# DanecLacey/basic_iterative_solvers

Hardware: AMD Instinct MI355X
Metric: CG iterations/sec + SpMV GFLOP/s (% HBM roofline), HPCG 256^3 at 1/2/4/8 GPUs (higher is better)
Workload: dtype f64

## Files before the change

### basic_iterative_solvers_amd/csrc/bis_blas1.hip

```cpp
#include "bis_internal.hpp"

#include <algorithm>
#include <cstdlib>

namespace {

constexpr int kEwThreads = 256;
constexpr int kMaxEwBlocks = 16384;

inline int ew_grid(int64_t n_items) {
    int64_t g = (n_items + kEwThreads - 1) / kEwThreads;
    if (g < 1) g = 1;
    if (g > kMaxDotBlocks) g = kMaxDotBlocks;
    return (int)g;
}
inline int ew_grid_wide(int64_t n_items) {
    int64_t g = (n_items + kEwThreads - 1) / kEwThreads;
    if (g < 1) g = 1;
    if (g > kMaxEwBlocks) g = kMaxEwBlocks;
    return (int)g;
}

typedef double ew_v2d_t __attribute__((ext_vector_type(2)));
__device__ __forceinline__ double2 ld_stream(const double2 *p) {
// ... 130 lines not shown
    int64_t i = (int64_t)blockIdx.x * kEwThreads + threadIdx.x;
    double acc0 = 0.0, acc1 = 0.0;
    if (VEC) {
        const int64_t n2 = n >> 1;
        double2 *w2 = reinterpret_cast<double2 *>(w);
        const double2 *u2 = reinterpret_cast<const double2 *>(u);
        const double2 *v2 = reinterpret_cast<const double2 *>(v);
        for (; i < n2; i += stride) {
            double2 wv = ld_stream(w2 + i);
            const double2 uv = ld_stream(u2 + i);
            wv.x = ew_apply<OP_SUB>(wv.x, uv.x, s);
            wv.y = ew_apply<OP_SUB>(wv.y, uv.y, s);
            w2[i] = wv;
            const double2 vv = v ? ld_stream(v2 + i) : wv;
            acc0 = fma(wv.x, vv.x, acc0);
            acc1 = fma(wv.y, vv.y, acc1);
        }
        if ((n & 1) && blockIdx.x == 0 && threadIdx.x == 0) {
            const double t = ew_apply<OP_SUB>(w[n - 1], u[n - 1], s);
            w[n - 1] = t;
            acc0 = fma(t, v ? v[n - 1] : t, acc0);
        }
    } else {
        for (; i < n; i += stride) {
            const double t = ew_apply<OP_SUB>(w[i], u[i], s);
            w[i] = t;
            acc0 = fma(t, v ? v[i] : t, acc0);
        }
    }
    const double r = block_sum<kEwThreads>(acc0 + acc1, lds);
    if (threadIdx.x == 0) partials[blockIdx.x] = r;
}

__global__ __launch_bounds__(256) void reduce_finish_kernel(const double *partials,
                                                            int n_partials, size_t stride,
                                                            double *result) {
    __shared__ double lds[4];
    const double *p = partials + (size_t)blockIdx.x * stride;
    double acc = 0.0;
    for (int i = threadIdx.x; i < n_partials; i += 256) acc += p[i];
    const double s = block_sum<256>(acc, lds);
    if (threadIdx.x == 0) result[blockIdx.x] = s;
}

enum { SC_DIV, SC_RATIO_PRODUCT, SC_SQRT_INV };
__global__ void scalar_kernel(int op, double *out, double *out2, const double *a, const double *b, const double *c,
                              const double *d) {
    if (op == SC_DIV) *out = *a / *b;
    else if (op == SC_RATIO_PRODUCT) *out = (*a / *b) * (*c / *d);
    else { const double nrm = sqrt(*a); *out = nrm; *out2 = 1.0 / nrm; }
}

}

bis_status bis_reduce_finish(bis_ctx *ctx, int n_partials, int n_values, size_t stride,
                             double *result_dev) {
    hipLaunchKernelGGL(reduce_finish_kernel, dim3(n_values), dim3(256), 0, ctx->stream,
                       ctx->partials, n_partials, stride, result_dev);
    BIS_HIP_CHECK(ctx, hipGetLastError());
    return BIS_OK;
}

bis_status bis_ensure_partials(bis_ctx *ctx, size_t n) {
    if (n <= ctx->partials_cap) return BIS_OK;
    BIS_HIP_CHECK(ctx, hipStreamSynchronize(ctx->stream));
    if (ctx->partials) BIS_HIP_CHECK(ctx, hipFree(ctx->partials));
    ctx->partials = nullptr;
    ctx->partials_cap = 0;
    BIS_HIP_CHECK(ctx, hipMalloc(&ctx->partials, sizeof(double) * n));
    ctx->partials_cap = n;
    return BIS_OK;
}

bis_status bis_fault_check(bis_ctx *ctx) {
    volatile unsigned *f = ctx->fault_host;
    if (!f || *f == 0) return BIS_OK;
    *f = 0;
    ctx->err = "a triangular sweep lost a hand-off: a row waited for a result that was never published "
               "(a workgroup of the persistent grid could not become resident, or the dependency data is corrupt); "
               "the vectors written since the last blocking call are invalid";
    return BIS_ERR_SYNC;
}

#define BIS_OPTIONS_ENV(X) X(spmv_variant) X(spmv_window) X(spmv_chunk) X(spmv_chunk_fused) X(spmv_xcd_remap) X(trsv_grid) X(ilu0_wgs) X(trsv_wave_wgs) X(trsv_trial) X(trsv_one_xcd) X(trsv_host_analysis) X(ilu0_wave) X(spmv_packed) X(spmv_packed32) X(spmv_valdict) X(spmv_sellwin) X(device_share) X(spmv_sellwin_rows) X(spmv_sellwin_joint) X(spmv_sellwin_pairs) X(spmv_sellwin_masks) X(spmv_colslab) X(spmv_win8) X(spmv_win8_rows) X(spmv_win8_depth) X(spmv_win8_implicit) X(spmv_win8_tune) X(spmv_win4) X(grid_autodetect) X(tune_placement) X(force_rp64) X(trsv_tiled) X(trsv_chain) X(trsv_tile_rows) X(trsv_tile_wgs) X(trsv_tile_edge) X(trsv_tile_backoff)
#define BIS_OPTIONS_API(Y) Y(trsv_batch) Y(trsv_wave) Y(ilu0_persistent) Y(trsv_by_pos) Y(spmv_lds_pad) Y(trsv_chain_idle) Y(trsv_chain_pause) Y(trsv_chain_pairs) Y(trsv_chain_prefix) Y(trsv_tile_exp) Y(cg_nt_x) Y(spmv_sellwin_nt) Y(dist_host_plan) Y(trsv_inject_loss) Y(trsv_inject_oom) Y(trsm_form)

namespace {
std::string &opts_env_seen() { static std::string s; return s; }
std::string upper_env(const char *name) {
    std::string e = "BIS_";
    for (const char *c = name; *c; ++c) e += (char)((*c >= 'a' && *c <= 'z') ? *c - 32 : *c);
    return e;
}
}

bis_options &bis_opts() {
    static bis_options o = [] {
        bis_options v;
#define X(name) { const std::string en = upper_env(#name); if (const char *e = getenv(en.c_str())) { v.name = atoi(e); \
                  std::string &seen = opts_env_seen(); if (!seen.empty()) seen += ' '; seen += en + "=" + e; } }
        BIS_OPTIONS_ENV(X)
#undef X
        return v;
    }();
    return o;
}

extern "C" {

bis_status bis_set_option(const char *name, int value) {
    if (!name) return BIS_ERR_INVALID;
    bis_options &o = bis_opts();
#define X(opt) if (!strcmp(name, #opt)) { o.opt = value; return BIS_OK; }
    BIS_OPTIONS_ENV(X)
    BIS_OPTIONS_API(X)
#undef X
    return BIS_ERR_INVALID;
}

int bis_options_describe(char *buf, int cap) {
    const bis_options &o = bis_opts();
    std::string s = "{";
    bool first = true;
#define X(opt) if (o.opt != -1) { if (!first) s += ", "; first = false; s += std::string("\"") + #opt + "\": " + std::to_string(o.opt); }
    BIS_OPTIONS_ENV(X)
    BIS_OPTIONS_API(X)
#undef X
    if (!first) s += ", ";
    s += "\"env\": \"";
    for (char c : opts_env_seen()) if (c != '"' && c != '\\' && (unsigned char)c >= 32) s += c;
    s += "\"}";
    if (buf && cap > 0) { const int n = std::min((int)s.size(), cap - 1); memcpy(buf, s.data(), (size_t)n); buf[n] = 0; }
    return (int)s.size();
}

int bis_abi_version(void) { return 1; }

bis_status bis_ctx_create(int device, void *stream, bis_ctx **out) {
    if (!out) return BIS_ERR_INVALID;
    *out = nullptr;
    int count = 0;
    if (hipGetDeviceCount(&count) != hipSuccess || count <= 0) return BIS_ERR_NO_DEVICE;
    if (device < 0 || device >= count) return BIS_ERR_NO_DEVICE;
    if (hipSetDevice(device) != hipSuccess) return BIS_ERR_NO_DEVICE;
    hipDeviceProp_t prop;
    if (hipGetDeviceProperties(&prop, device) != hipSuccess) return BIS_ERR_NO_DEVICE;
    bis_ctx *ctx = new bis_ctx;
    ctx->device = device;
    ctx->n_cus = prop.multiProcessorCount;
    ctx->arch = prop.gcnArchName;
    ctx->hbm_bytes = (int64_t)prop.totalGlobalMem;
    if (ctx->arch.rfind("gfx950", 0) != 0) {
        fprintf(stderr, "bis_hip: device %d is %s, this library is built for gfx950 only\n",
                device, ctx->arch.c_str());
        delete ctx;
        return BIS_ERR_NO_DEVICE;
    }
    if (stream) {
        ctx->stream = (hipStream_t)stream;
    } else {
        if (hipStreamCreateWithFlags(&ctx->stream, hipStreamNonBlocking) != hipSuccess) {
            delete ctx;
            return BIS_ERR_HIP;
        }
        ctx->own_stream = true;
    }
    ctx->partials_cap = std::max((size_t)kMaxReduceBlocks * 4, (size_t)kMaxDotBlocks * 2);
// ... 327 lines not shown
```

### basic_iterative_solvers_amd/csrc/bis_internal.hpp

```cpp
#pragma once

#include <hip/hip_runtime.h>

#include <cstdint>
#include <cstdio>
#include <cstring>
#include <map>
#include <string>
#include <vector>

#include "bis_hip.h"

struct bis_trsv_plan;
struct bis_trsv_tiled;
struct bis_trsv_chain;
struct bis_trsm_plan;
struct bis_trsv_side {
    bis_trsv_plan *level = nullptr;
    bis_trsv_tiled *tiled = nullptr;
    bis_trsv_chain *chain = nullptr;
    bis_trsm_plan *multi = nullptr;
    bool tiled_tried = false, chain_tried = false;
    const char *kernel = "";
    const char *kernel_m = "";
// ... 3 lines not shown
    int type = 0;
    const bis_mat *A = nullptr;
    double *B = nullptr, *C = nullptr;
    int64_t size_B = 0, size_C = 0;
    const double *D = nullptr;
    bool upper = false;
};

struct bis_ctx {
    int device = 0;
    hipStream_t stream = nullptr;
    bool own_stream = false;
    int n_cus = 0;
    std::string arch;
    int64_t hbm_bytes = 0;
    std::string err;

    double *partials = nullptr;
    size_t partials_cap = 0;
    double *scalars_dev = nullptr;
    double *scalars_host = nullptr;
    unsigned *counters = nullptr;
    unsigned *fault_host = nullptr, *fault_dev = nullptr;

    std::map<std::string, bis_named_kernel> kernels;

    const int *spmv_stop = nullptr;

    bool profile = false;
    std::vector<std::pair<hipEvent_t, hipEvent_t>> prof_events;
    size_t prof_used = 0;
    std::vector<std::pair<hipEvent_t, hipEvent_t>> prof_sweep_events;
    size_t prof_sweep_used = 0;
};

struct bis_options;
bis_options &bis_opts();
struct bis_options {
    int spmv_variant = -1;
    int spmv_window = -1;
    int spmv_chunk = -1;
    int spmv_chunk_fused = -1;
    int spmv_xcd_remap = -1;
    int trsv_grid = -1;
    int ilu0_wave = -1;
    int ilu0_wgs = -1;
    int ilu0_persistent = -1;
    int trsv_host_analysis = -1;
    int trsv_wave = -1;
    int trsv_wave_wgs = -1;
    int trsv_trial = -1;
    int trsv_batch = -1;
    int trsv_by_pos = -1;
    int trsv_one_xcd = -1;
    int tune_placement = -1;
    int spmv_packed32 = -1;
    int spmv_lds_pad = -1;
    int spmv_packed = -1;
    int spmv_valdict = -1;
    int dist_host_plan = -1;
    int grid_autodetect = -1;
    int trsv_chain = -1;
    int trsv_chain_idle = -1;
    int trsv_chain_pause = -1;
    int trsv_chain_prefix = -1;
    int trsv_chain_pairs = -1;
    int trsv_tiled = -1;
    int trsv_tile_rows = -1;
    int trsv_tile_wgs = -1;
    int trsv_tile_backoff = -1;
    int spmv_sellwin_nt = -1;
    int cg_nt_x = -1;
    int trsv_tile_exp = -1;
    int trsv_tile_edge = -1;
    int force_rp64 = -1;
    int spmv_sellwin = -1;
    int spmv_sellwin_rows = -1;
    int spmv_sellwin_pairs = -1;
    int spmv_sellwin_joint = -1;
    int spmv_colslab = -1;
    int spmv_win8 = -1;
    int spmv_win8_rows = -1;
    int spmv_win8_depth = -1;
    int spmv_win8_implicit = -1;
    int spmv_win8_tune = -1;
    int spmv_win4 = -1;
    int spmv_sellwin_masks = -1;
    int device_share = -1;
    int trsm_form = -1;
    int trsv_inject_oom = -1;
    int trsv_inject_loss = -1;
};
inline bool bis_want_rp64(int64_t nnz) { return nnz >= (int64_t)INT32_MAX - 8 || bis_opts().force_rp64 > 0; }

constexpr int kMaxReduceBlocks = 2048;
constexpr int kMaxDotBlocks = 8192;
constexpr int kWinMaxTiles = 128;
constexpr int kWinTile = 16;
constexpr int kWinTileLog = 4;
constexpr int kSwRows = 256;
constexpr int kSwMaxR = 4;

struct bis_mat {
    int64_t n_rows = 0, n_cols = 0, nnz = 0;
    bool rp64 = false;
    bool view = false;
    void *row_ptr = nullptr;
    int32_t *col = nullptr;
    double *val = nullptr;
    int32_t *blk_row = nullptr;
    int64_t *blk_nnz = nullptr;
    uint16_t *loc = nullptr;
    int32_t *tiles = nullptr;
    int32_t *tile_cnt = nullptr;
    int64_t loc_base = 0;
    int max_tiles = 0;
    bool win_ok = false;
    int n_blocks = 0;
    uint16_t *pk[2] = {nullptr, nullptr};
    int32_t *pk_seg[2] = {nullptr, nullptr};
    int64_t pk_base[2] = {0, 0};
    int pk_state[2] = {0, 0};
    int pk_kind[2] = {0, 0};
    uint8_t *vcode = nullptr;
    double *vdict = nullptr;
    int64_t vd_base = 0;
    int vd_state = 0, vd_n = 0;
    double *vdiag = nullptr;
    bool vd_diag = false;
    bool vd_rm_only = false;
    int64_t view_row0 = 0;
    int64_t *rm_nnz = nullptr;
    uint16_t *rm_pk = nullptr;
    int32_t *rm_seg = nullptr;
    int64_t rm_base = 0;
    int rm_state = 0, rm_blocks = 0, rm_kind = 1;
    struct bis_sellwin *sw = nullptr;
    int sw_state = 0;
    struct bis_sellwin *sw8 = nullptr;
    std::vector<bis_mat *> *colslabs = nullptr;
    int cs_state = 0;
    double cs_trial_ms[2] = {0.0, 0.0};
    int sw8_state = 0;
    struct bis_sellwin *sw4 = nullptr;
    int sw4_state = 0;
    bool f32_exact = false;
    int32_t *blkf_row = nullptr;
    int64_t *blkf_nnz = nullptr;
    int n_blocks_f = 0;
    int chunk_f = 0;
    int chunk_nnz = 0;
    int max_row_nnz = 0;
    int64_t max_block_nnz = 0;
    int64_t grid[4] = {0, 0, 0, 0};
    bis_trsv_side trsv[2];
    const char *spmv_kernel[2] = {"", ""};
    const char *ilu0_kernel = "";
    const char *itrsv_kernel = "";
    const char *spmm_kernel = "";
    const char *fsai_kernel = "";
    struct bis_mg *mg = nullptr;
};

#define BIS_HIP_CHECK(ctx, call)                                               \
    do {                                                                       \
        hipError_t e_ = (call);                                                \
// ... 175 lines not shown
```

### basic_iterative_solvers_amd/csrc/bis_spmv_sell.hip

```cpp
#include <algorithm>
#include <cstring>
#include <cstdio>
#include <cstdlib>
#include <vector>

#include <rocprim/rocprim.hpp>

#include "bis_internal.hpp"

struct bis_sellwin {
    int n_blocks = 0;
    int64_t n_slices = 0, total_chunks = 0;
    int32_t *hdr = nullptr;
    int64_t *slice_chunk0 = nullptr;
    int32_t *own_rank = nullptr;
    uint32_t *codes = nullptr;
    double *dict = nullptr;
    int max_gran = 0;
    int fmt = 0;
    int uniform_chunks = 0;
    int n_pairs = 0, pair_stride = 0, diag_pair = -1;
    int16_t *blk_base = nullptr;
    unsigned long long *pair_key = nullptr;
    uint16_t *row_of = nullptr;
    void *own_codes = nullptr;
    size_t w8_desc = 0, w8_side = 0, w8_end = 0;
    int64_t *slice_rec = nullptr;
    int64_t expl_chunks = 0;
    int64_t win_gran_sum = 0;
    int tune_trials = 0;
    double tune_first_ms = 0.0, tune_kept_ms = 0.0;
    int R = 1;
    int vb = 8;
    bool diag = false;
    int pad_idx = 0, diag_idx = 0;
};

namespace {

constexpr int kSwRuns = 32;
constexpr int kSwRunGran = 64;
constexpr int kSwHash = 4096;
constexpr int kSwMaxGran = 940;
constexpr int kSwDefaultR = 2;
constexpr int kSwMaxPairs = 253;
inline int sw_gran_cap(int R) { return R == 4 ? kSwMaxGran : std::min(kSwMaxGran, (65536 - (4096 + 4096 * R) - 16) / 64); }

__device__ __forceinline__ unsigned long long sw_pair_key(int32_t offset, unsigned vcode) {
    return ((unsigned long long)((unsigned)offset ^ 0x80000000u) << 8) | vcode;
}

__device__ __forceinline__ int sw_wave_max(int v) {
    for (int o = 32; o > 0; o >>= 1) v = max(v, __shfl_xor(v, o));
    return v;
}

template <typename RP>
__global__ __launch_bounds__(256) void sw_plan_kernel(const RP *__restrict__ row_ptr, const int32_t *__restrict__ col,
                                                      int64_t n_rows, int R, int max_gran, int64_t row0, int32_t *__restrict__ hdr,
                                                      int32_t *__restrict__ slice_chunks, int32_t *__restrict__ own_rank, int *status) {
    __shared__ int table[kSwHash];
    __shared__ int list[1024];
    __shared__ int cnt, n_runs, failed;
    __shared__ int run_g0[kSwRuns], run_rank[kSwRuns], srt_g0[kSwRuns], srt_rank[kSwRuns + 1];
    const int b = blockIdx.x, tid = threadIdx.x;
    const int64_t r0 = (int64_t)b * kSwRows * R;
    const int rows = (int)min((int64_t)kSwRows * R, n_rows - r0);
    for (int i = tid; i < kSwHash; i += 256) table[i] = -1;
    if (tid == 0) { cnt = 0; n_runs = 0; failed = 0; }
    __syncthreads();
    for (int r = 0; r < R; ++r) {
        const int sl = (tid >> 6) * R + r, lr = sl * 64 + (tid & 63);
        int len = 0;
        if (lr < rows) len = (int)((int64_t)row_ptr[r0 + lr + 1] - (int64_t)row_ptr[r0 + lr]);
        const int m = sw_wave_max(len);
        if ((tid & 63) == 0) { slice_chunks[(size_t)b * 4 * R + sl] = (m + 3) >> 2; atomicMax(&status[5], (m + 3) >> 2); }
    }
    const int64_t s = (int64_t)row_ptr[r0], e = (int64_t)row_ptr[r0 + rows];
    for (int64_t k = s + tid; k < e; k += 256) {
        if (__hip_atomic_load(&failed, __ATOMIC_RELAXED, __HIP_MEMORY_SCOPE_WORKGROUP)) break;
        const int g = col[k] >> 3;
        unsigned h = ((unsigned)g * 2654435761u) >> 20;
        for (;;) {
            const int cur = __hip_atomic_load(&table[h], __ATOMIC_RELAXED, __HIP_MEMORY_SCOPE_WORKGROUP);
            if (cur == g) break;
            if (cur == -1) {
// ... 1245 lines not shown
                    *reinterpret_cast<float4 *>(p + 512 + lane * 16) = make_float4((float)vv[0], (float)vv[1], (float)vv[2], (float)vv[3]);
                } else {
                    *reinterpret_cast<double2 *>(p + 512 + lane * 16) = make_double2(vv[0], vv[1]);
                    *reinterpret_cast<double2 *>(p + 1536 + lane * 16) = make_double2(vv[2], vv[3]);
                }
            } else {
                unsigned char *p = stream + (size_t)(c0 + c) * w8_val_bytes<VT>();
                if constexpr (sizeof(VT) == 4) {
                    *reinterpret_cast<float4 *>(p + lane * 16) = make_float4((float)vv[0], (float)vv[1], (float)vv[2], (float)vv[3]);
                } else {
                    *reinterpret_cast<double2 *>(p + lane * 16) = make_double2(vv[0], vv[1]);
                    *reinterpret_cast<double2 *>(p + 1024 + lane * 16) = make_double2(vv[2], vv[3]);
                }
                if (!implicit) *reinterpret_cast<uint2 *>(side + (size_t)(slice_rec[slice] + c) * 512 + lane * 8) = make_uint2(cc[0] | cc[1] << 16, cc[2] | cc[3] << 16);
                else if (lane == 0) desc[c0 + c] = make_uint2(base[0] | base[1] << 16, base[2] | base[3] << 16);
            }
        }
        if (PHASE == 1 && lane == 0) slice_rec[slice] = implicit ? 0 : nch;
    }
}

typedef double w8_v2d __attribute__((ext_vector_type(2)));
typedef unsigned w8_v2u __attribute__((ext_vector_type(2)));
typedef float w8_v4f __attribute__((ext_vector_type(4)));
template <typename VT> struct W8Chunk { w8_v2u code; w8_v2d v0, v1; };
template <> struct W8Chunk<float> { w8_v2u code; w8_v4f v; };

template <typename VT>
__device__ __forceinline__ W8Chunk<VT> w8_load(const unsigned char *__restrict__ stream, int64_t c, int lane) {
    const unsigned char *p = stream + (size_t)c * w8_chunk_bytes<VT>();
    W8Chunk<VT> ch;
    ch.code = __builtin_nontemporal_load(reinterpret_cast<const w8_v2u *>(p + lane * 8));
    if constexpr (sizeof(VT) == 4) {
        ch.v = __builtin_nontemporal_load(reinterpret_cast<const w8_v4f *>(p + 512 + lane * 16));
    } else {
        ch.v0 = __builtin_nontemporal_load(reinterpret_cast<const w8_v2d *>(p + 512 + lane * 16));
        ch.v1 = __builtin_nontemporal_load(reinterpret_cast<const w8_v2d *>(p + 1536 + lane * 16));
    }
    return ch;
}

template <typename VT>
__device__ __forceinline__ void w8_load_values(const unsigned char *__restrict__ stream, int64_t c, int lane, W8Chunk<VT> &ch) {
    const unsigned char *p = stream + (size_t)c * w8_val_bytes<VT>();
    if constexpr (sizeof(VT) == 4) {
        ch.v = __builtin_nontemporal_load(reinterpret_cast<const w8_v4f *>(p + lane * 16));
    } else {
        ch.v0 = __builtin_nontemporal_load(reinterpret_cast<const w8_v2d *>(p + lane * 16));
        ch.v1 = __builtin_nontemporal_load(reinterpret_cast<const w8_v2d *>(p + 1024 + lane * 16));
    }
}

typedef unsigned short w8_v2h __attribute__((ext_vector_type(2)));
__device__ __forceinline__ unsigned w8_imply(unsigned code, unsigned off2) {
    const unsigned pad = (code & 0x10001u) * 0xffffu;
    return __builtin_bit_cast(unsigned, __builtin_bit_cast(w8_v2h, code) + __builtin_bit_cast(w8_v2h, off2)) & ~pad;
}

__device__ __forceinline__ void w8_consume(const unsigned char *win, const W8Chunk<double> &ch, double &acc) {
#pragma clang fp contract(off)
    const double x0 = *reinterpret_cast<const double *>(win + (ch.code.x & 0xffffu));
    const double x1 = *reinterpret_cast<const double *>(win + (ch.code.x >> 16));
    const double x2 = *reinterpret_cast<const double *>(win + (ch.code.y & 0xffffu));
    const double x3 = *reinterpret_cast<const double *>(win + (ch.code.y >> 16));
    const double p0 = ch.v0.x * x0, p1 = ch.v0.y * x1, p2 = ch.v1.x * x2, p3 = ch.v1.y * x3;
    acc = acc + p0;
    acc = acc + p1;
    acc = acc + p2;
    acc = acc + p3;
}
__device__ __forceinline__ void w8_consume(const unsigned char *win, const W8Chunk<float> &ch, double &acc) {
#pragma clang fp contract(off)
    const double x0 = *reinterpret_cast<const double *>(win + (ch.code.x & 0xffffu));
    const double x1 = *reinterpret_cast<const double *>(win + (ch.code.x >> 16));
    const double x2 = *reinterpret_cast<const double *>(win + (ch.code.y & 0xffffu));
    const double x3 = *reinterpret_cast<const double *>(win + (ch.code.y >> 16));
    const double p0 = (double)ch.v.x * x0, p1 = (double)ch.v.y * x1, p2 = (double)ch.v.z * x2, p3 = (double)ch.v.w * x3;
    acc = acc + p0;
    acc = acc + p1;
    acc = acc + p2;
    acc = acc + p3;
}

template <int MODE, int R, int D, bool IMPL, typename VT = double>
__global__ __launch_bounds__(256) void spmv_win8_kernel(
    const double *x, double *__restrict__ y, int64_t n_rows, int64_t n_cols, int n_blocks, int remap_arg, const double *w,
    double *__restrict__ partials, const int *stop, const int32_t *__restrict__ hdr, const int64_t *__restrict__ slice_chunk0,
    const unsigned char *__restrict__ stream, int x_al16, const int32_t *__restrict__ own_rank, const uint16_t *__restrict__ row_of,
    const w8_v2u *__restrict__ desc, const unsigned char *__restrict__ side, const int64_t *__restrict__ slice_rec) {
    if (stop && stop[1]) return;
    extern __shared__ __attribute__((aligned(16))) unsigned char lds[];
    const int b = remap_arg > 0 ? xcd_remap(blockIdx.x, remap_arg)
                                : (remap_arg < -1 ? xcd_group_remap(blockIdx.x, -remap_arg) : (int)blockIdx.x);
    if (b >= n_blocks) return;
    const int tid = threadIdx.x, lane = tid & 63;
    const int wv = __builtin_amdgcn_readfirstlane(tid >> 6);
    const int hw_g = hdr[(size_t)b * 2 * kW8Runs + lane], hw_r = hdr[(size_t)b * 2 * kW8Runs + kW8Runs + lane];
    const int64_t slice0 = ((int64_t)b * 4 + wv) * R;
    const int64_t block_row0 = (int64_t)b * kSwRows * R;
    int64_t rows_of[R];
#pragma unroll
    for (int r = 0; r < R; ++r) rows_of[r] = block_row0 + row_of[(slice0 + r) * 64 + lane];
    const int64_t my_bnd = slice_chunk0[slice0 + min(lane, R)];
    auto bnd = [&](int r) {
        const unsigned lo = (unsigned)__builtin_amdgcn_readlane((int)(unsigned)(unsigned long long)my_bnd, r);
        const unsigned hi = (unsigned)__builtin_amdgcn_readlane((int)(unsigned)((unsigned long long)my_bnd >> 32), r);
        return (int64_t)(((unsigned long long)hi << 32) | lo);
    };
    const int64_t C0 = bnd(0), C1 = bnd(R);
    const int64_t c_last = max(C1 - 1, C0);
    int64_t e[R];
#pragma unroll
    for (int rr = 0; rr < R; ++rr) e[rr] = bnd(rr + 1);
    int64_t rec[R + 1];
    unsigned off2[R];
    if (IMPL) {
        const int64_t my_rec = slice_rec[slice0 + min(lane, R)];
#pragma unroll
        for (int r = 0; r <= R; ++r) {
            const unsigned lo = (unsigned)__builtin_amdgcn_readlane((int)(unsigned)(unsigned long long)my_rec, r);
            const unsigned hi = (unsigned)__builtin_amdgcn_readlane((int)(unsigned)((unsigned long long)my_rec >> 32), r);
            rec[r] = (int64_t)(((unsigned long long)hi << 32) | lo);
        }
#pragma unroll
        for (int r = 0; r < R; ++r) off2[r] = rec[r + 1] == rec[r] ? (unsigned)(rows_of[r] - block_row0) * 0x80008u : 0u;
    }
    auto load = [&](int64_t cc) {
        if (!IMPL) return w8_load<VT>(stream, cc, lane);
        W8Chunk<VT> ch;
        w8_load_values<VT>(stream, cc, lane, ch);
        int64_t rs = 0, re = 0, cs = 0;
#pragma unroll
        for (int rr = 0; rr < R; ++rr)
            if (cc >= (rr ? e[rr - 1] : C0) && cc < e[rr]) { rs = rec[rr]; re = rec[rr + 1]; cs = rr ? e[rr - 1] : C0; }
        if (re > rs) ch.code = __builtin_nontemporal_load(reinterpret_cast<const w8_v2u *>(side + (size_t)(rs + cc - cs) * 512 + lane * 8));
        else ch.code = desc[cc];
        return ch;
    };
    W8Chunk<VT> ring[D];
#pragma unroll
    for (int d = 0; d < D; ++d) ring[d] = load(min(C0 + d, c_last));
    double wr[R];
    int own = -1;
    if (MODE == 1 && own_rank) own = own_rank[b];
#pragma unroll
    for (int r = 0; r < R; ++r) {
        const int64_t row = rows_of[r];
        wr[r] = (MODE == 1 && own < 0 && row < n_rows) ? w[row] : 0.0;
    }
    if (tid == 0) *reinterpret_cast<double *>(lds) = -0.0;
    {
        const int n_runs = __popcll(__ballot((hw_r >> 16) != 0));
        unsigned char *win = lds + 16;
        for (int k = 0; k < n_runs; ++k) {
            const int g0 = __builtin_amdgcn_readlane(hw_g, k);
            const int w2 = __builtin_amdgcn_readlane(hw_r, k);
            const int rank = w2 & 0xffff, n_pieces = (w2 >> 16) * 4;
            const int j = (wv + k) & 3;
            const int p = j * 64 + lane;
            const int64_t c = (int64_t)g0 * 8 + 2 * p;
            unsigned char *dst = win + (size_t)rank * 64 + (size_t)j * 1024;
            if (p < n_pieces) {
                if (x_al16 && c + 1 < n_cols) {
                    __builtin_amdgcn_global_load_lds((const __attribute__((address_space(1))) void *)(x + c),
                                                     (__attribute__((address_space(3))) void *)dst, 16, 0, 0);
                } else {
                    double2 v;
                    v.x = c < n_cols ? x[c] : 0.0;
                    v.y = c + 1 < n_cols ? x[c + 1] : 0.0;
                    *reinterpret_cast<double2 *>(dst + lane * 16) = v;
                }
            }
        }
    }
    __syncthreads();
    if (MODE == 1 && own >= 0) {
#pragma unroll
        for (int r = 0; r < R; ++r) wr[r] = *reinterpret_cast<const double *>(lds + 16 + ((size_t)own * 8 + (wv * R + r) * 64 + lane) * 8);
    }
    double dot_acc = 0.0;
    int64_t c = C0;
    int next = 0;
    double acc = 0.0;
    unsigned cur_off = IMPL ? off2[0] : 0u;
#define W8_END_SLICES()                                                                    \
    _Pragma("unroll") for (int rr = 0; rr < R; ++rr)                                       \
        if (rr == next && c == e[rr]) {                                                    \
            const int64_t row = rows_of[rr];                                               \
            if (row < n_rows) y[row] = acc;                                                \
            if (MODE == 1) dot_acc += row < n_rows ? acc * wr[rr] : 0.0;                   \
            acc = 0.0;                                                                     \
            ++next;                                                                        \
            if (IMPL) cur_off = off2[rr + 1 < R ? rr + 1 : R - 1];                         \
        }
    W8_END_SLICES()
    while (c < C1) {
#pragma unroll
        for (int d = 0; d < D; ++d) {
            if (c < C1) {
                W8Chunk<VT> cur = ring[d];
                ring[d] = load(min(c + D, c_last));
                if (IMPL) {
                    cur.code.x = w8_imply(cur.code.x, cur_off);
                    cur.code.y = w8_imply(cur.code.y, cur_off);
                }
                w8_consume(lds, cur, acc);
                ++c;
                W8_END_SLICES()
            }
        }
    }
#undef W8_END_SLICES
    if (MODE == 1) {
        const double t = wave_sum(dot_acc);
        if (lane == 0) partials[(size_t)b * 4 + wv] = t;
    }
}

}

static inline bis_sellwin *&w8_ptr(bis_mat *A, int vb) { return vb == 4 ? A->sw4 : A->sw8; }
static inline int &w8_state(bis_mat *A, int vb) { return vb == 4 ? A->sw4_state : A->sw8_state; }
static inline const bis_sellwin *w8_get(const bis_mat *A, int vb) {
    return (vb == 4 ? A->sw4_state : A->sw8_state) == 1 ? (vb == 4 ? A->sw4 : A->sw8) : nullptr;
}

static void w8_drop_one(bis_mat *A, int vb) {
    if (bis_sellwin *&sw = w8_ptr(A, vb)) {
        if (sw->own_codes) sw->codes = reinterpret_cast<uint32_t *>(sw->own_codes);
        hipFree(sw->hdr); hipFree(sw->slice_chunk0); hipFree(sw->own_rank); hipFree(sw->codes); hipFree(sw->row_of);
        hipFree(sw->slice_rec);
        delete sw;
        sw = nullptr;
    }
    w8_state(A, vb) = 0;
}

void bis_spmv_win8_drop(bis_mat *A) {
    w8_drop_one(A, 8);
    w8_drop_one(A, 4);
}

int bis_spmv_win8_active(const bis_mat *A) {
    return A->f32_exact && A->sw4_state == 1 && bis_opts().spmv_win4 != 0 && bis_opts().spmv_win8 != 0 ? 4 : 8;
}

int bis_spmv_win8_blocks(const bis_mat *A, int vb) { const bis_sellwin *sw = w8_get(A, vb); return sw ? sw->n_blocks : 0; }
int bis_spmv_win8_rows(const bis_mat *A, int vb) { const bis_sellwin *sw = w8_get(A, vb); return sw ? sw->R : 0; }
bool bis_spmv_win8_implied(const bis_mat *A, int vb) { const bis_sellwin *sw = w8_get(A, vb); return sw && sw->slice_rec != nullptr; }
int64_t bis_spmv_win8_bytes(const bis_mat *A, int vb) {
    const bis_sellwin *sw = w8_get(A, vb);
    if (!sw) return 0;
    const int64_t meta = (int64_t)sw->n_blocks * (8 * kW8Runs + 2 * kSwRows * sw->R) + 8 * (sw->n_slices + 1);
    if (!sw->slice_rec) return sw->total_chunks * (int64_t)w8_chunk_bytes(vb) + meta;
    return sw->total_chunks * (int64_t)w8_val_bytes(vb) + 8 * (sw->total_chunks - sw->expl_chunks) + 512 * sw->expl_chunks + meta + 8 * (sw->n_slices + 1);
}

size_t bis_spmv_win8_stream_bytes(const bis_mat *A, int vb) {
    const bis_sellwin *sw = w8_get(A, vb);
    if (!sw) return 0;
    return sw->slice_rec ? sw->w8_end : w8_chunk_bytes(vb) * (size_t)(sw->total_chunks + 1);
}

double bis_spmv_win8_moved_bytes(const bis_mat *A, int vb) {
    const bis_sellwin *sw = w8_get(A, vb);
    if (!sw) return 0.0;
    return (double)bis_spmv_win8_bytes(A, vb) + 64.0 * (double)sw->win_gran_sum + 8.0 * (double)A->n_rows;
}
bool bis_spmv_win8_fast(const bis_mat *A, double ms, int vb) {
    return w8_get(A, vb) && ms > 0.0 && bis_spmv_win8_moved_bytes(A, vb) / (ms * 1e-3) >= 6.6e12;
}
void *bis_spmv_win8_swap_stream(bis_mat *A, void *stream, int vb) {
    bis_sellwin *sw = w8_ptr(A, vb);
    void *old = sw->codes;
    sw->codes = reinterpret_cast<uint32_t *>(stream);
    return old;
}

#define W8_CHECK(call)                                                         \
    do {                                                                       \
        hipError_t e_ = (call);                                                \
        if (e_ != hipSuccess) {                                                \
            (void)hipGetLastError();                                           \
            hipFree(slice_chunks); hipFree(tmp);                               \
            w8_drop_one(A, vb);                                                \
            w8_state(A, vb) = -1;                                              \
            if (e_ == hipErrorOutOfMemory) return BIS_OK;  \
            ctx->err = std::string(#call) + ": " + hipGetErrorString(e_);      \
            return BIS_ERR_HIP;                                                \
        }                                                                      \
    } while (0)

static bis_status w8_tune_placement(bis_ctx *ctx, bis_mat *A, int vb) {
    bis_sellwin *sw = w8_ptr(A, vb);
    const size_t bytes = bis_spmv_win8_stream_bytes(A, vb);
// ... 133 lines not shown
    W8_CHECK(hipMemcpyAsync(h, status, sizeof h, hipMemcpyDeviceToHost, ctx->stream));
    const int64_t ns1 = sw->n_slices + 1;
    hipLaunchKernelGGL(sw_widen_kernel, dim3((unsigned)((ns1 + 255) / 256)), dim3(256), 0, ctx->stream, slice_chunks, sw->slice_chunk0, ns1);
    W8_CHECK(hipGetLastError());
    size_t tmp_bytes = 0;
    W8_CHECK(rocprim::exclusive_scan(nullptr, tmp_bytes, sw->slice_chunk0, sw->slice_chunk0, (int64_t)0, (size_t)ns1, rocprim::plus<int64_t>(), ctx->stream));
    W8_CHECK(hipMalloc(&tmp, tmp_bytes));
    W8_CHECK(rocprim::exclusive_scan(tmp, tmp_bytes, sw->slice_chunk0, sw->slice_chunk0, (int64_t)0, (size_t)ns1, rocprim::plus<int64_t>(), ctx->stream));
    int64_t total = 0;
    W8_CHECK(hipMemcpyAsync(&total, sw->slice_chunk0 + sw->n_slices, sizeof total, hipMemcpyDeviceToHost, ctx->stream));
    W8_CHECK(hipStreamSynchronize(ctx->stream));
    hipFree(tmp); tmp = nullptr;
    hipFree(slice_chunks); slice_chunks = nullptr;
    sw->total_chunks = total;
    sw->max_gran = h[1];
    sw->win_gran_sum = (int64_t)(unsigned)h[2];
    if (h[0] || (double)total * 256.0 > 1.12 * (double)A->nnz + 256.0 * 4 * 64) {
        if (getenv("BIS_WIN8_STATS")) fprintf(stderr, "win8 plan (R = %d): %s, %.1f %% padding: not used\n", R, h[0] ? "window not representable" : "representable", 100.0 * ((double)total * 256.0 / (double)A->nnz - 1.0));
        *window_too_large = h[0] != 0;
        w8_drop_one(A, vb);
        w8_state(A, vb) = -1;
        return BIS_OK;
    }
#define W8_FILL(PHASE, VT, STREAM, DESC, SIDE)                                                                                                    \
    do {                                                                                                                                          \
        if (A->rp64) hipLaunchKernelGGL((w8_fill_kernel<int64_t, PHASE, VT>), dim3(nb), dim3(256), 0, ctx->stream, (const int64_t *)A->row_ptr, A->col, \
                                        A->val, A->n_rows, R, sw->hdr, sw->slice_chunk0, sw->row_of, STREAM, sw->slice_rec, DESC, SIDE);           \
        else hipLaunchKernelGGL((w8_fill_kernel<int32_t, PHASE, VT>), dim3(nb), dim3(256), 0, ctx->stream, (const int32_t *)A->row_ptr, A->col, \
                                A->val, A->n_rows, R, sw->hdr, sw->slice_chunk0, sw->row_of, STREAM, sw->slice_rec, DESC, SIDE);                   \
        W8_CHECK(hipGetLastError());                                                                                                              \
    } while (0)
    sw->expl_chunks = total;
    if (bis_opts().spmv_win8_implicit != 0 && total > 0) {
        W8_CHECK(hipMalloc(&sw->slice_rec, sizeof(int64_t) * (size_t)ns1));
        W8_CHECK(hipMemsetAsync(sw->slice_rec, 0, sizeof(int64_t) * (size_t)ns1, ctx->stream));
        W8_FILL(1, double, nullptr, nullptr, nullptr);
        tmp_bytes = 0;
        W8_CHECK(rocprim::exclusive_scan(nullptr, tmp_bytes, sw->slice_rec, sw->slice_rec, (int64_t)0, (size_t)ns1, rocprim::plus<int64_t>(), ctx->stream));
        W8_CHECK(hipMalloc(&tmp, tmp_bytes));
        W8_CHECK(rocprim::exclusive_scan(tmp, tmp_bytes, sw->slice_rec, sw->slice_rec, (int64_t)0, (size_t)ns1, rocprim::plus<int64_t>(), ctx->stream));
        int64_t expl = 0;
        W8_CHECK(hipMemcpyAsync(&expl, sw->slice_rec + sw->n_slices, sizeof expl, hipMemcpyDeviceToHost, ctx->stream));
        W8_CHECK(hipStreamSynchronize(ctx->stream));
        hipFree(tmp); tmp = nullptr;
        if (2 * (total - expl) >= total) sw->expl_chunks = expl;
        else { hipFree(sw->slice_rec); sw->slice_rec = nullptr; }
    }
    unsigned char *stream = nullptr;
    const size_t chunk_bytes = sw->slice_rec ? w8_val_bytes(vb) : w8_chunk_bytes(vb);
    size_t stream_bytes = chunk_bytes * (size_t)(total + 1);
    if (sw->slice_rec) {
        sw->w8_desc = stream_bytes;
        sw->w8_side = sw->w8_desc + ((8 * (size_t)(total + 1) + 255) & ~(size_t)255);
        sw->w8_end = stream_bytes = sw->w8_side + 512 * (size_t)sw->expl_chunks;
    }
    W8_CHECK(hipMalloc(&stream, stream_bytes));
    sw->codes = reinterpret_cast<uint32_t *>(stream);
    W8_CHECK(hipMemsetAsync(stream + (size_t)total * chunk_bytes, 0, chunk_bytes, ctx->stream));
    if (sw->slice_rec) {
        W8_CHECK(hipMemsetAsync(stream + sw->w8_desc, 0, sw->w8_side - sw->w8_desc, ctx->stream));
        if (vb == 4) W8_FILL(2, float, stream, reinterpret_cast<uint2 *>(stream + sw->w8_desc), stream + sw->w8_side);
        else W8_FILL(2, double, stream, reinterpret_cast<uint2 *>(stream + sw->w8_desc), stream + sw->w8_side);
    } else {
        if (vb == 4) W8_FILL(0, float, stream, nullptr, nullptr);
        else W8_FILL(0, double, stream, nullptr, nullptr);
    }
#undef W8_FILL
    w8_state(A, vb) = 1;
    if (bis_status tst = w8_tune_placement(ctx, A, vb)) return tst;
    if (getenv("BIS_WIN8_STATS")) fprintf(stderr, "win%d plan (R = %d): %d blocks, window <= %d granules (%zu bytes), %.1f %% padding: used; implied slots: %s, %.1f %% of %lld chunks implicit; stream at %p (%zu bytes), hdr %p\n", vb, R, nb, sw->max_gran, (size_t)(2 + 8 * sw->max_gran) * 8, 100.0 * ((double)total * 256.0 / (double)A->nnz - 1.0), sw->slice_rec ? "built" : "not built", 100.0 * (double)(total - sw->expl_chunks) / (double)std::max<int64_t>(total, 1), (long long)total, (void *)sw->codes, bis_spmv_win8_stream_bytes(A, vb), (void *)sw->hdr);
    return BIS_OK;
}
#undef W8_CHECK

bis_status bis_spmv_win8_launch(bis_ctx *ctx, const bis_mat *A, const double *x, double *y, int mode, const double *w,
                                double *partials, const int *stop, int remap_arg, int grid, int vb) {
    const bis_sellwin *sw = vb == 4 ? A->sw4 : A->sw8;
    const int x_al16 = ((uintptr_t)x & 15) == 0;
    const size_t lds = (size_t)(2 + 8 * sw->max_gran) * 8;
    const unsigned char *stream = reinterpret_cast<const unsigned char *>(sw->codes);
    const int32_t *own = (mode == 1 && w == x + A->view_row0 && x_al16) ? sw->own_rank : nullptr;
    const bool ragged = (double)sw->total_chunks * 256.0 > 1.08 * (double)A->nnz;
    const int depth = bis_opts().spmv_win8_depth > 0 ? bis_opts().spmv_win8_depth : (sw->R == 4 ? (ragged ? 2 : 1) : 3);
#define W8_L3(MODE, RR, DD) do { if (sw->slice_rec) W8_L5(MODE, RR, DD, true); else W8_L5(MODE, RR, DD, false); } while (0)
#define W8_L5(MODE, RR, DD, IMPL) do { if (vb == 4) W8_L4(MODE, RR, DD, IMPL, float); else W8_L4(MODE, RR, DD, IMPL, double); } while (0)
#define W8_L4(MODE, RR, DD, IMPL, VT) hipLaunchKernelGGL((spmv_win8_kernel<MODE, RR, DD, IMPL, VT>), dim3(grid), dim3(256), lds, ctx->stream, x, y, A->n_rows, A->n_cols, \
                                               sw->n_blocks, remap_arg, w, partials, stop, sw->hdr, sw->slice_chunk0, stream, x_al16, own, sw->row_of, \
                                               reinterpret_cast<const w8_v2u *>(stream + sw->w8_desc), stream + sw->w8_side, sw->slice_rec)
#define W8_L2(MODE, RR) do { if (depth <= 1) W8_L3(MODE, RR, 1); else if (depth == 2) W8_L3(MODE, RR, 2); else if (depth == 3) W8_L3(MODE, RR, 3); else if (depth <= 5) W8_L3(MODE, RR, 4); else W8_L3(MODE, RR, 6); } while (0)
#define W8_L1(MODE) do { if (sw->R == 4) W8_L2(MODE, 4); else if (sw->R == 2) W8_L2(MODE, 2); else W8_L2(MODE, 1); } while (0)
    if (mode == 1) W8_L1(1); else W8_L1(0);
#undef W8_L1
#undef W8_L2
#undef W8_L3
#undef W8_L4
#undef W8_L5
    BIS_HIP_CHECK(ctx, hipGetLastError());
    return BIS_OK;
}
```

Measured before the change: 1064.

## Add slice-nested chunk walk to win8 SpMV kernel for depth-1 prefetch

Adds a NEST template variant of the windowed SELL SpMV kernel that walks chunks per owned row-slice in a nested loop. It prefetches one chunk ahead with the slot-format decision hoisted per slice, instead of checking slice boundaries on every chunk in a flat loop. It becomes the default whenever the chosen prefetch depth is 1, and an env option can override it. The aim is to cut per-chunk branching and index bookkeeping in the inner loop. The cost is extra template instantiations and code size, and possible register pressure from the lambdas.

```diff
diff --git a/basic_iterative_solvers_amd/csrc/bis_blas1.hip b/basic_iterative_solvers_amd/csrc/bis_blas1.hip
--- a/basic_iterative_solvers_amd/csrc/bis_blas1.hip
+++ b/basic_iterative_solvers_amd/csrc/bis_blas1.hip
@@ -236,7 +236,7 @@
     return BIS_ERR_SYNC;
 }
 
-#define BIS_OPTIONS_ENV(X) X(spmv_variant) X(spmv_window) X(spmv_chunk) X(spmv_chunk_fused) X(spmv_xcd_remap) X(trsv_grid) X(ilu0_wgs) X(trsv_wave_wgs) X(trsv_trial) X(trsv_one_xcd) X(trsv_host_analysis) X(ilu0_wave) X(spmv_packed) X(spmv_packed32) X(spmv_valdict) X(spmv_sellwin) X(device_share) X(spmv_sellwin_rows) X(spmv_sellwin_joint) X(spmv_sellwin_pairs) X(spmv_sellwin_masks) X(spmv_colslab) X(spmv_win8) X(spmv_win8_rows) X(spmv_win8_depth) X(spmv_win8_implicit) X(spmv_win8_tune) X(spmv_win4) X(grid_autodetect) X(tune_placement) X(force_rp64) X(trsv_tiled) X(trsv_chain) X(trsv_tile_rows) X(trsv_tile_wgs) X(trsv_tile_edge) X(trsv_tile_backoff)
+#define BIS_OPTIONS_ENV(X) X(spmv_variant) X(spmv_window) X(spmv_chunk) X(spmv_chunk_fused) X(spmv_xcd_remap) X(trsv_grid) X(ilu0_wgs) X(trsv_wave_wgs) X(trsv_trial) X(trsv_one_xcd) X(trsv_host_analysis) X(ilu0_wave) X(spmv_packed) X(spmv_packed32) X(spmv_valdict) X(spmv_sellwin) X(device_share) X(spmv_sellwin_rows) X(spmv_sellwin_joint) X(spmv_sellwin_pairs) X(spmv_sellwin_masks) X(spmv_colslab) X(spmv_win8) X(spmv_win8_rows) X(spmv_win8_depth) X(spmv_win8_walk) X(spmv_win8_implicit) X(spmv_win8_tune) X(spmv_win4) X(grid_autodetect) X(tune_placement) X(force_rp64) X(trsv_tiled) X(trsv_chain) X(trsv_tile_rows) X(trsv_tile_wgs) X(trsv_tile_edge) X(trsv_tile_backoff)
 #define BIS_OPTIONS_API(Y) Y(trsv_batch) Y(trsv_wave) Y(ilu0_persistent) Y(trsv_by_pos) Y(spmv_lds_pad) Y(trsv_chain_idle) Y(trsv_chain_pause) Y(trsv_chain_pairs) Y(trsv_chain_prefix) Y(trsv_tile_exp) Y(cg_nt_x) Y(spmv_sellwin_nt) Y(dist_host_plan) Y(trsv_inject_loss) Y(trsv_inject_oom) Y(trsm_form)
 
 namespace {
diff --git a/basic_iterative_solvers_amd/csrc/bis_internal.hpp b/basic_iterative_solvers_amd/csrc/bis_internal.hpp
--- a/basic_iterative_solvers_amd/csrc/bis_internal.hpp
+++ b/basic_iterative_solvers_amd/csrc/bis_internal.hpp
@@ -109,6 +109,7 @@
     int spmv_win8 = -1;
     int spmv_win8_rows = -1;
     int spmv_win8_depth = -1;
+    int spmv_win8_walk = -1;
     int spmv_win8_implicit = -1;
     int spmv_win8_tune = -1;
     int spmv_win4 = -1;
diff --git a/basic_iterative_solvers_amd/csrc/bis_spmv_sell.hip b/basic_iterative_solvers_amd/csrc/bis_spmv_sell.hip
--- a/basic_iterative_solvers_amd/csrc/bis_spmv_sell.hip
+++ b/basic_iterative_solvers_amd/csrc/bis_spmv_sell.hip
@@ -2,6 +2,7 @@
 #include <cstring>
 #include <cstdio>
 #include <cstdlib>
+#include <type_traits>
 #include <vector>
 
 #include <rocprim/rocprim.hpp>
@@ -1413,12 +1414,13 @@
     acc = acc + p3;
 }
 
-template <int MODE, int R, int D, bool IMPL, typename VT = double>
+template <int MODE, int R, int D, bool IMPL, typename VT = double, bool NEST = false>
 __global__ __launch_bounds__(256) void spmv_win8_kernel(
     const double *x, double *__restrict__ y, int64_t n_rows, int64_t n_cols, int n_blocks, int remap_arg, const double *w,
     double *__restrict__ partials, const int *stop, const int32_t *__restrict__ hdr, const int64_t *__restrict__ slice_chunk0,
     const unsigned char *__restrict__ stream, int x_al16, const int32_t *__restrict__ own_rank, const uint16_t *__restrict__ row_of,
     const w8_v2u *__restrict__ desc, const unsigned char *__restrict__ side, const int64_t *__restrict__ slice_rec) {
+    static_assert(!NEST || D == 1, "the slice-nested walk requests one chunk ahead");
     if (stop && stop[1]) return;
     extern __shared__ __attribute__((aligned(16))) unsigned char lds[];
     const int b = remap_arg > 0 ? xcd_remap(blockIdx.x, remap_arg)
@@ -1510,6 +1512,63 @@
         for (int r = 0; r < R; ++r) wr[r] = *reinterpret_cast<const double *>(lds + 16 + ((size_t)own * 8 + (wv * R + r) * 64 + lane) * 8);
     }
     double dot_acc = 0.0;
+    if constexpr (NEST) {
+        constexpr unsigned CB = IMPL ? (unsigned)w8_val_bytes<VT>() : (unsigned)w8_chunk_bytes<VT>();
+        const int nC = (int)(C1 - C0), k_last = max(nC - 1, 0);
+        int le[R];
+#pragma unroll
+        for (int rr = 0; rr < R; ++rr) le[rr] = (int)(e[rr] - C0);
+        const unsigned char *vp = stream + (size_t)C0 * CB + lane * 16 + (IMPL ? 0 : 512);
+        const w8_v2u *dp = desc + (IMPL ? C0 : 0);
+        auto values = [&](int kk, W8Chunk<VT> &ch) {
+            const unsigned char *p = vp + (unsigned)kk * CB;
+            if constexpr (!IMPL) ch.code = __builtin_nontemporal_load(reinterpret_cast<const w8_v2u *>(p - 512 - lane * 8));
+            if constexpr (sizeof(VT) == 4) {
+                ch.v = __builtin_nontemporal_load(reinterpret_cast<const w8_v4f *>(p));
+            } else {
+                ch.v0 = __builtin_nontemporal_load(reinterpret_cast<const w8_v2d *>(p));
+                ch.v1 = __builtin_nontemporal_load(reinterpret_cast<const w8_v2d *>(p + 1024));
+            }
+        };
+        W8Chunk<VT> cur = ring[0];
+        int k = 0;
+        double acc = 0.0;
+#pragma unroll
+        for (int rr = 0; rr < R; ++rr) {
+            const int ls = rr ? le[rr - 1] : 0, end = le[rr];
+            const bool expl = IMPL && rec[rr + 1] != rec[rr];
+            auto slots = [&](auto FL, int kk, const unsigned char *sp, W8Chunk<VT> &ch) {
+                if constexpr (FL.value == 1) ch.code = dp[kk];
+                if constexpr (FL.value == 2) ch.code = __builtin_nontemporal_load(reinterpret_cast<const w8_v2u *>(sp + ((unsigned)(kk - ls) << 9)));
+            };
+            auto consume = [&](auto FL, unsigned off, W8Chunk<VT> &ch) {
+                if constexpr (FL.value == 1) {
+                    ch.code.x = w8_imply(ch.code.x, off);
+                    ch.code.y = w8_imply(ch.code.y, off);
+                }
+                w8_consume(lds, ch, acc);
+            };
+            auto slice = [&](auto FL, const unsigned char *sp, unsigned off) {
+                if (FL.value != 0 && rr > 0 && k < end) slots(FL, k, sp, cur);
+                while (k < end) {
+                    W8Chunk<VT> nxt;
+                    nxt.code = cur.code;
+                    values(min(k + 1, k_last), nxt);
+                    if (k + 1 < end) slots(FL, k + 1, sp, nxt);
+                    consume(FL, off, cur);
+                    cur = nxt;
+                    ++k;
+                }
+            };
+            if constexpr (!IMPL) slice(std::integral_constant<int, 0>(), nullptr, 0u);
+            else if (expl) slice(std::integral_constant<int, 2>(), side + (size_t)rec[rr] * 512 + lane * 8, 0u);
+            else slice(std::integral_constant<int, 1>(), nullptr, off2[rr]);
+            const int64_t row = rows_of[rr];
+            if (row < n_rows) y[row] = acc;
+            if (MODE == 1) dot_acc += row < n_rows ? acc * wr[rr] : 0.0;
+            acc = 0.0;
+        }
+    } else {
     int64_t c = C0;
     int next = 0;
     double acc = 0.0;
@@ -1542,6 +1601,7 @@
         }
     }
 #undef W8_END_SLICES
+    }
     if (MODE == 1) {
         const double t = wave_sum(dot_acc);
         if (lane == 0) partials[(size_t)b * 4 + wv] = t;
@@ -1841,12 +1901,13 @@
     const int32_t *own = (mode == 1 && w == x + A->view_row0 && x_al16) ? sw->own_rank : nullptr;
     const bool ragged = (double)sw->total_chunks * 256.0 > 1.08 * (double)A->nnz;
     const int depth = bis_opts().spmv_win8_depth > 0 ? bis_opts().spmv_win8_depth : (sw->R == 4 ? (ragged ? 2 : 1) : 3);
-#define W8_L3(MODE, RR, DD) do { if (sw->slice_rec) W8_L5(MODE, RR, DD, true); else W8_L5(MODE, RR, DD, false); } while (0)
-#define W8_L5(MODE, RR, DD, IMPL) do { if (vb == 4) W8_L4(MODE, RR, DD, IMPL, float); else W8_L4(MODE, RR, DD, IMPL, double); } while (0)
-#define W8_L4(MODE, RR, DD, IMPL, VT) hipLaunchKernelGGL((spmv_win8_kernel<MODE, RR, DD, IMPL, VT>), dim3(grid), dim3(256), lds, ctx->stream, x, y, A->n_rows, A->n_cols, \
+    const bool nest = bis_opts().spmv_win8_walk >= 0 ? bis_opts().spmv_win8_walk != 0 : depth <= 1;
+#define W8_L3(MODE, RR, DD, NEST) do { if (sw->slice_rec) W8_L5(MODE, RR, DD, true, NEST); else W8_L5(MODE, RR, DD, false, NEST); } while (0)
+#define W8_L5(MODE, RR, DD, IMPL, NEST) do { if (vb == 4) W8_L4(MODE, RR, DD, IMPL, float, NEST); else W8_L4(MODE, RR, DD, IMPL, double, NEST); } while (0)
+#define W8_L4(MODE, RR, DD, IMPL, VT, NEST) hipLaunchKernelGGL((spmv_win8_kernel<MODE, RR, DD, IMPL, VT, NEST>), dim3(grid), dim3(256), lds, ctx->stream, x, y, A->n_rows, A->n_cols, \
                                                sw->n_blocks, remap_arg, w, partials, stop, sw->hdr, sw->slice_chunk0, stream, x_al16, own, sw->row_of, \
                                                reinterpret_cast<const w8_v2u *>(stream + sw->w8_desc), stream + sw->w8_side, sw->slice_rec)
-#define W8_L2(MODE, RR) do { if (depth <= 1) W8_L3(MODE, RR, 1); else if (depth == 2) W8_L3(MODE, RR, 2); else if (depth == 3) W8_L3(MODE, RR, 3); else if (depth <= 5) W8_L3(MODE, RR, 4); else W8_L3(MODE, RR, 6); } while (0)
+#define W8_L2(MODE, RR) do { if (nest) W8_L3(MODE, RR, 1, true); else if (depth <= 1) W8_L3(MODE, RR, 1, false); else if (depth == 2) W8_L3(MODE, RR, 2, false); else if (depth == 3) W8_L3(MODE, RR, 3, false); else if (depth <= 5) W8_L3(MODE, RR, 4, false); else W8_L3(MODE, RR, 6, false); } while (0)
 #define W8_L1(MODE) do { if (sw->R == 4) W8_L2(MODE, 4); else if (sw->R == 2) W8_L2(MODE, 2); else W8_L2(MODE, 1); } while (0)
     if (mode == 1) W8_L1(1); else W8_L1(0);
 #undef W8_L1
```

After: 1116 (median of 6 runs). +4.9%, better.
